# agimus-project/agimus_controller

Measured on AMD Instinct MI355X. Metric: MPC steps/sec (horizon=100, Panda 7-DoF), higher is better.
Workload: dtype f64; 1 GPU; Panda 7-DoF sine_wave_configuration_space, ocp_goal_reaching.yaml costs, horizon=100, dt=0.01, batch=1024 independent MPC instances per GPU (seed 1234+b), closed loop on own prediction; horizon=100, batch_per_gpu=1024, global_batch=1024, max_iter=10

## Files before the change

agimus_controller_amd/backend.py:

```python

from __future__ import annotations

import ctypes as C
import os
import pathlib
import subprocess

import numpy as np

from . import _abi

_CSRC = pathlib.Path(__file__).resolve().parent / "csrc"
LIB_PATH = pathlib.Path(os.environ.get("AGX_LIB", _CSRC / "libagimus_hip.so"))
NOGEN_LIB_PATH = _CSRC / "libagimus_hip_nogen.so"
_LIB = None

EXPORTED_SYMBOLS = [
    "agx_last_error", "agx_device_count", "agx_row_nref", "agx_row_nr", "agx_ref_stride",
    "agx_model_create", "agx_model_destroy", "agx_ocp_create", "agx_ocp_destroy", "agx_ocp_set_stream",
    "agx_ocp_sync", "agx_ocp_set_refs", "agx_ocp_set_refs_device", "agx_ocp_solve", "agx_ocp_upload_x0",
    "agx_ocp_upload_warmstart", "agx_ocp_solve_resident", "agx_ocp_download", "agx_ocp_download_first", "agx_ocp_first_packed", "agx_ocp_set_geom_placement", "agx_ocp_reset_duals", "agx_traj_generic_create", "agx_traj_set_horizon_indexes", "agx_ocp_feedback_rollout", "agx_ocp_download_x0", "agx_model_frame_jacobian",
    "agx_ocp_shift_warmstart", "agx_ocp_x0_from_prediction", "agx_ocp_integrate", "agx_model_rnea",
    "agx_model_frame_placement", "agx_ocp_get_residuals", "agx_ocp_calc_diff", "agx_ocp_direction",
    "agx_ocp_time_kernel", "agx_ocp_profile", "agx_traj_sine_create", "agx_traj_set_window",
    "agx_traj_get_point", "agx_traj_warmstart_from_reference", "agx_ocp_mpc_step", "agx_ocp_qp_tiles", "agx_ocp_set_quorum",
    "agx_traj_cartesian_sine_create", "agx_ocp_set_refs_async", "agx_ocp_refs_activate", "agx_ocp_refs_wait", "agx_host_alloc", "agx_host_free",
    "agx_ocp_download_async", "agx_ocp_download_wait",
    "agx_traj_generic_create_weighted", "agx_traj_cartesian_sine_wi_create", "agx_traj_get_tile",
    "agx_ocp_set_plant_inertials", "agx_model_sensitivity", "agx_ocp_cost_wide", "agx_ocp_set_model_inertials",
    "agx_traj_stream_create", "agx_traj_stream_append", "agx_traj_stream_release", "agx_traj_stream_range",
    "agx_traj_stream_joins", "agx_traj_stream_timing", "agx_ocp_set_obstacle_placements",
    "agx_ocp_set_first_pack", "agx_ocp_first_pack_counts", "agx_ocp_handoff_counts",
    "agx_ocp_iter_log", "agx_ocp_iter_log_read", "agx_ocp_item_costs", "agx_ocp_carry_counts", "agx_ocp_general_rows",
]


def _run(cmd, verbose):
    res = subprocess.run(cmd, capture_output=True, text=True)
    if verbose or res.returncode != 0:
        print(res.stdout, res.stderr)
    if res.returncode != 0:
        raise RuntimeError(f"{cmd[0]} failed ({res.returncode}): {res.stderr[-2000:]}")


def build(force: bool = False, verbose: bool = False) -> pathlib.Path:
    hdr = _CSRC.parent.parent / "include" / "agimus_hip.h"
    pairs_src = _CSRC / "agx_cost_pairs.hip"
    diag_src = _CSRC / "agx_diag.hip"
# ... 128 lines not shown
        self.nv = self.pm.nv
        self.nx, self.nu = 2 * self.nv, self.nv
        self.T, self.B = packed_ocp.horizon, int(batch)
        self.stride = packed_ocp.stride
        self.tile = _abi.tile_doubles(self.nv)
        self._log_cap = 0
        self._m = C.c_void_p()
        self._h = C.c_void_p()
        _chk(L.agx_model_create(C.byref(self.pm.desc), C.byref(self._m)))
        rc = L.agx_ocp_create(self._m, C.byref(self.po.desc), self.B, int(device), C.byref(self._h))
        if rc != 0:
            msg = L.agx_last_error().decode()
            L.agx_model_destroy(self._m)
            self._m = None
            raise HipError(msg)

    @property
    def cost_wide(self) -> bool:
        return lib().agx_ocp_cost_wide(self._h) == 1

    @property
    def general_rows(self) -> bool:
        return lib().agx_ocp_general_rows(self._h) == 1

    def close(self):
        if getattr(self, "_h", None):
            lib().agx_ocp_destroy(self._h)
            self._h = None
        if getattr(self, "_m", None):
            lib().agx_model_destroy(self._m)
# ... 95 lines not shown
        st = None
        if want_status:
            q = buf[:, nu + nk + nx:]
            names = ("kkt", "cost", "merit", "gap_norm", "iter", "qp_iters", "solved", "flags")
            if copy:
                st = np.zeros(self.B, dtype=_abi.STATUS_DTYPE)
                for k, name in enumerate(names):
                    st[name] = q[:, k] if k < 4 else q[:, k].astype(np.int32)
            else:
                st = {name: q[:, k] for k, name in enumerate(names)}
        return us0, K0, x1, st

    def set_first_pack(self, in_solve: bool = True):
        _chk(lib().agx_ocp_set_first_pack(self._h, 1 if in_solve else 0))

    def first_pack_counts(self):
        a, b = C.c_longlong(0), C.c_longlong(0)
        _chk(lib().agx_ocp_first_pack_counts(self._h, C.byref(a), C.byref(b)))
        return int(a.value), int(b.value)

    def handoff_counts(self):
        a, b = C.c_longlong(0), C.c_int(0)
        _chk(lib().agx_ocp_handoff_counts(self._h, C.byref(a), C.byref(b)))
        return int(a.value), int(b.value)

    def carry_counts(self):
        a, b = C.c_longlong(0), C.c_longlong(0)
        _chk(lib().agx_ocp_carry_counts(self._h, C.byref(a), C.byref(b)))
        return int(a.value), int(b.value)

# ... 280 lines not shown
```

agimus_controller_amd/csrc/agimus_hip.hip:

```cpp

#include <hip/hip_runtime.h>

#include <algorithm>
#include <chrono>
#include <climits>
#include <cmath>
#include <cstddef>
#include <cstdio>
#include <cstdlib>
#include <cstring>
#include <string>
#include <vector>

#include "agx_kernels.hpp"

extern "C" int agx_cost_pairs_launch(int dest, void *stream, long long nodes, const DevModel *m, const DevOcp *o, const DevCostWide *w,
                                     const double *dts, const double *xs, const RefView *rv, double *out, double *auxs, const DevState *st,
                                     int phase, int sel, int which, const void *obs);
extern "C" int agx_cost_pairs_fill_launch(void *stream, const DevCostWide *w, const double *gw_item, double *traj, long long units, int stride);
extern "C" int agx_cost_pairs_fill_ring_launch(void *stream, const DevCostWide *w, const double *gw_item, double *traj, int B, int m_new, int end,
                                               int cap, int mirror, int stride);
extern "C" int agx_diag_iter_log_launch(void *stream, const DevState *st, int B, int it, int phase, agx_iter_record *rec, int *n, int capacity);
extern "C" int agx_diag_item_costs_launch(void *stream, int nv, int chain, const DevModel *m, const DevRows *rows2, int B, int T, const double *xs,
                                          const double *us, const RefView *rv, int R, double *cost, double *Lx, double *Lu, const void *obs);
// ... 321 lines not shown
  if (kGeneralRowsWg && o->general && o->nv > 7 && !term_only) {
    const double *xs_in = phase ? o->d_xs + (size_t)o->B * (o->T + 1) * o->nx : o->d_xs;
    const double *us_in = phase ? o->d_us + (size_t)o->B * o->T * o->nu : o->d_us;
    HIPCHK((hipError_t)agx_general_rows_launch(kGenToQp, (void *)o->stream, o->nv, o->hm.prismatic ? 1 : 0, (long long)o->B * (o->T + 1), o->d_model,
                                               o->d_ocp, o->d_dt, xs_in, us_in, &o->rv, o->d_qt, o->d_aux, o->d_auxg, o->d_state, phase, -1, 0));
  }
  return o->cost_wide ? launch_cost_pairs(o, agx::kPairsToQp, running_only ? 1 : (term_only ? 2 : 0), phase) : 0;
}

template <int NV>
void launch_riccati_blk(agx_ocp *o, const double *tiles, int forward, int gains_pass) {
  hipLaunchKernelGGL((agx::k_riccati_blk<NV>), dim3(o->B), dim3(256), 0, o->stream, o->d_ocp, o->d_dt, tiles, o->d_Kws, o->d_kws, o->d_dx,
                     o->d_w, o->d_state, forward, gains_pass);
}

int launch_riccati(agx_ocp *o, int forward, bool pair = false, int iter = 0, const double *tiles = nullptr) {
  if (o->nv <= 7 && o->T + 1 > 512) return fail("the sweeps stage the step lengths of up to 511 nodes in LDS: horizon too long");
  return dispatch(o->nv, o->chain, [&](auto NVc, auto CHc) -> int {
    constexpr int NV = decltype(NVc)::value;
    const double *qt = tiles ? tiles : o->d_qt;
    if constexpr (NV <= 7) if (o->mx2_S >= 2 && o->riccati_mx && !tiles) {
      const int S = o->mx2_S, P2 = pair ? 2 : 1;
      if (!o->d_mx2_elem) {
        HIPCHK(o->own.device(&o->d_mx2_elem, 2 * (size_t)o->B * S * 768));
        HIPCHK(o->own.device(&o->d_mx2_bnd, 2 * (size_t)o->B * S * 256));
        HIPCHK(o->own.device(&o->d_mx2_cl, (size_t)o->B * S * 256));
      }
      hipLaunchKernelGGL((agx::k_riccati_mx2_elem<NV>), dim3(P2 * o->B * S), dim3(64), 0, o->stream, o->d_ocp, o->d_dt, o->d_qt, o->d_aux,
                         o->d_Kws, o->d_kws, o->d_Kout, o->d_state, o->d_mx2_elem, o->d_mx2_bnd, o->d_mx2_cl, S, pair ? 1 : 0, 0, 1, iter);
      hipLaunchKernelGGL((agx::k_riccati_mx2_sweep<NV>), dim3(P2 * o->B * (S - 1)), dim3(64), 0, o->stream, o->d_ocp, o->d_dt, o->d_qt, o->d_aux,
                         o->d_Kws, o->d_kws, o->d_Kout, o->d_state, o->d_mx2_elem, o->d_mx2_bnd, o->d_mx2_cl, S, pair ? 1 : 0, 0, 1);
      if (forward)
        hipLaunchKernelGGL((agx::k_riccati_mx2_fwd<NV>), dim3(o->B * S), dim3(64), 0, o->stream, o->d_ocp, o->d_dt, o->d_qt, o->d_Kws, o->d_kws,
                           o->d_dx, o->d_w, o->d_state, o->d_mx2_cl, S);
      HIPCHK(hipGetLastError());
      return 0;
    }
    if constexpr (NV <= 7) {
      if (pair && o->riccati_mx)
        hipLaunchKernelGGL((agx::k_riccati_mx_pair<NV>), dim3(16 * ((o->B + 7) / 8)), dim3(64), 0, o->stream, o->d_ocp, o->d_dt, o->d_qt, o->d_aux,
                           o->d_Kws, o->d_kws, o->d_dx, o->d_w, o->d_Kout, o->d_state, iter);
      else if (pair)
        hipLaunchKernelGGL((agx::k_riccati_pair<NV>), dim3(2 * o->B), dim3(64), 0, o->stream, o->d_ocp, o->d_dt, o->d_qt, o->d_aux,
                           o->d_Kws, o->d_kws, o->d_dx, o->d_w, o->d_du, o->d_Kout, o->d_state, iter);
      else if (o->riccati_mx)
        hipLaunchKernelGGL((agx::k_riccati_mx<NV, false>), dim3(o->B), dim3(64), 0, o->stream, o->d_ocp, o->d_dt, qt, o->d_aux,
                           o->d_Kws, o->d_kws, o->d_dx, o->d_w, o->d_Kout, o->d_state, forward, 0);
      else
        hipLaunchKernelGGL((agx::k_riccati<NV, false>), dim3(o->B), dim3(64), 0, o->stream, o->d_ocp, o->d_dt, qt, o->d_aux,
                           o->d_Kws, o->d_kws, o->d_dx, o->d_w, o->d_du, o->d_Kout, o->d_state, forward, 0);
    } else {
      (void)pair; (void)iter;
      launch_riccati_blk<NV>(o, qt, forward, 0);
    }
    HIPCHK(hipGetLastError());
    return 0;
  });
}

agx::HostWords host_words(agx_ocp *o, bool line_search_counters, unsigned long long seq) {
  agx::HostWords hw{nullptr, nullptr, nullptr, nullptr, nullptr, nullptr, 0};
  if (!o->poll || !o->fold_publish || seq == 0) return hw;
  hw.done = o->h_ndone_dev + 0;
  if (line_search_counters) { hw.handed = o->h_ndone_dev + 6; hw.stale = o->h_ndone_dev + 7; }
  hw.carry = o->h_ndone_dev + 8;
  hw.packed = o->h_ndone_dev + 9;
  hw.seq = o->h_ndone_dev + 1;
  hw.stamp = seq;
  return hw;
}

double *first_block(const agx_ocp *o) {
  return (o->first_in_solve && o->poll && o->first_stride == o->nu + o->nu * o->nx + o->nx + 8) ? o->d_first : nullptr;
}

int launch_step(agx_ocp *o, int iter, int max_iter, int mode, bool with_node_kkt = true, bool with_step = true, unsigned long long seq = 0,
                bool pack = false) {
  if (o->T + 1 > 512) return fail("step kernel supports horizons up to 511 nodes");
  return dispatch(o->nv, o->chain, [&](auto NVc, auto CHc) -> int {
    constexpr int NV = decltype(NVc)::value;
    constexpr bool CH = decltype(CHc)::value;
    (void)CH;
    const long long nodes = (long long)o->B * (o->T + 1);
    double *xs_t = o->d_xs + (size_t)o->B * (o->T + 1) * o->nx, *us_t = o->d_us + (size_t)o->B * o->T * o->nu;
    if (with_node_kkt) {
      if constexpr (NV <= 7) {
        if (o->general)
          hipLaunchKernelGGL((agx::k_node_kkt_gen<NV>), dim3((int)((nodes + 63) / 64)), dim3(64), 0, o->stream, o->d_ocp, o->d_qt, o->d_aux,
                             o->d_auxg, o->d_dx, o->d_w, o->d_du, o->d_nodestat, o->d_state);
        else if (o->node_kkt_wide)
          hipLaunchKernelGGL((agx::k_node_kkt_ahead<NV>), dim3((int)((nodes + 7) / 8)), dim3(64), 0, o->stream, o->d_ocp, o->d_qt, o->d_aux,
                             o->d_dx, o->d_w, o->d_du, o->d_nodestat, o->d_state);
        else
          hipLaunchKernelGGL((agx::k_node_kkt<NV>), dim3((int)((nodes * 8 + 255) / 256)), dim3(256), 0, o->stream, o->d_ocp, o->d_qt, o->d_aux,
                             o->d_dx, o->d_w, o->d_du, o->d_nodestat, o->d_state);
      } else if (kGeneralRowsWg && o->general)
        HIPCHK((hipError_t)agx_general_kkt_launch((void *)o->stream, NV, nodes, o->d_ocp, o->d_qt, o->d_aux, o->d_auxg, o->d_dx, o->d_w, o->d_du,
                                                  o->d_nodestat, o->d_state));
      else
        hipLaunchKernelGGL((agx::k_node_kkt_big<NV>), dim3((int)((nodes + 1) / 2)), dim3(64), 0, o->stream, o->d_ocp, o->d_qt, o->d_aux,
                           o->d_dx, o->d_w, o->d_du, o->d_nodestat, o->d_state);
    }
    if (with_step)
      hipLaunchKernelGGL((agx::k_sqp_head<NV>), dim3(o->B), dim3(128), 0, o->stream, o->d_ocp, o->d_xs, o->d_us, o->d_dx, o->d_du, xs_t, us_t,
                         o->d_nodestat, o->d_state, iter, max_iter, mode, o->d_ndone, host_words(o, false, seq), o->d_Kout,
                         pack ? first_block(o) : nullptr, o->first_stride);
    HIPCHK(hipGetLastError());
    return 0;
  });
}

int launch_gains(agx_ocp *o, int gmode = 0) {
  if (o->nv <= 7 && o->T + 1 > 512) return fail("the sweeps stage the step lengths of up to 511 nodes in LDS: horizon too long");
  if (o->nv > 7 && !o->d_qt2) HIPCHK(o->own.device(&o->d_qt2, (size_t)o->B * (o->T + 1) * o->qt_size));
  return dispatch(o->nv, o->chain, [&](auto NVc, auto CHc) -> int {
    constexpr int NV = decltype(NVc)::value;
    if constexpr (NV <= 7) {
      if (o->riccati_mx)
        hipLaunchKernelGGL((agx::k_riccati_mx<NV, true>), dim3(o->B), dim3(64), 0, o->stream, o->d_ocp, o->d_dt, o->d_qt, o->d_aux, o->d_Kws,
                           o->d_kws, o->d_dx, o->d_w, o->d_Kout, o->d_state, 0, gmode);
      else
// ... 398 lines not shown
    if (need_k1) {
      if (it == 0 && carry_mode != 0) {
        if (launch_calc_qp(o, false, false, 0, carry_mode == 2)) return -1;
      } else if (o->prof && it == 0) {
        if (prof_mark(o, 0, true)) return -1;
        if (launch_calc_qp(o, true, false)) return -1;
        if (prof_mark(o, 0, false)) return -1;
        if (launch_calc_qp(o, false, true)) return -1;
      } else if (launch_calc_qp(o, false, false)) return -1;
    }
    need_k1 = false;
    if (prof_mark(o, 1, true)) return -1;
    if (o->has_con && o->admm_prefactor && o->riccati_mx && o->nv <= 7 && !o->general) {
      if (admm_direction(o, true)) return -1;
    } else {
      if (launch_riccati(o, 1, pair, it)) return -1;
      if (o->has_con && admm_direction(o)) return -1;
    }
    if (prof_mark(o, 1, false)) return -1;
    const bool last = it + 1 == max_iter;
    if (prof_mark(o, 2, true)) return -1;
    const unsigned long long seq_head = ++o->seq;
    if (launch_step(o, it, max_iter, 1, !o->has_con, true, seq_head, pair && packing)) return -1;
    if (prof_mark(o, 2, false)) return -1;
    if (iter_log_mark(o, it, 0)) return -1;
    unsigned long long seq_early = 0;
    if (o->poll && !o->fold_publish && !o->prof && !o->no_empty && it >= 1) {
      seq_early = ++o->seq;
      hipLaunchKernelGGL(agx::k_publish3, dim3(1), dim3(1), 0, o->stream, o->d_ndone, o->h_ndone_dev + 11, (unsigned long long *)nullptr, (unsigned long long *)nullptr, o->h_ndone_dev + 12,
                         o->h_ndone_dev + 13, o->h_ndone_dev + 10, seq_early);
      HIPCHK(hipGetLastError());
    }
    int n_done = 0;
    if (!pair && !o->has_con && (last || max_time > 0.0 || o->quorum_sqp < 1.0)) {
      if (launch_gains(o, 4)) return -1;
    }
    bool searching = true;
    if (o->poll && o->fold_publish && it >= 1) {
// ... 780 lines not shown
    if (st) {
      const double *q = r + nu + nk + nx;
      st[b].kkt = q[0]; st[b].cost = q[1]; st[b].merit = q[2]; st[b].gap_norm = q[3];
      st[b].iter = (int)q[4]; st[b].qp_iters = (int)q[5]; st[b].solved = (int)q[6]; st[b].flags = (int)q[7];
    }
  }
  return 0;
}

int agx_ocp_set_first_pack(agx_ocp *o, int in_solve) {
  if (!o) return fail("null handle");
  o->first_in_solve = in_solve != 0;
  return 0;
}

int agx_ocp_first_pack_counts(agx_ocp *o, long long *served_in_solve, long long *served_by_launch) {
  if (!o) return fail("null handle");
  if (served_in_solve) *served_in_solve = o->first_served[0];
  if (served_by_launch) *served_by_launch = o->first_served[1];
  return 0;
}

int agx_ocp_handoff_counts(agx_ocp *o, long long *early_exits, int *n_carriable) {
  if (!o) return fail("null handle");
  if (early_exits) *early_exits = o->early_exits;
  if (n_carriable) *n_carriable = o->n_carriable;
  return 0;
}

int agx_ocp_carry_counts(agx_ocp *o, long long *steps_carried, long long *steps_full) {
// ... 302 lines not shown
  if (launch_step(o, 0, 1, 0)) return -1;
  if (launch_gains(o)) return -1;
  const size_t B = o->B, T = o->T, nx = o->nx, nu = o->nu;
  (void)nx; (void)nu;
  if (K && down_gains(o, K, o->d_Kout, B * T)) return -1;
  if (k && down(o, k, o->d_kws, B * T, 1)) return -1;
  if (dx && down(o, dx, o->d_dx, B * (T + 1), 2)) return -1;
  if (du && down(o, du, o->d_du, B * T, 1)) return -1;
  std::vector<DevState> hs(B);
  HIPCHK(hipMemcpyAsync(hs.data(), o->d_state, sizeof(DevState) * B, hipMemcpyDeviceToHost, o->stream));
  HIPCHK(hipStreamSynchronize(o->stream));
  if (kkt) for (size_t b = 0; b < B; ++b) kkt[b] = hs[b].kkt;
  return 0;
}

int agx_ocp_qp_tiles(agx_ocp *o, double *qt, double *aux, int *qt_size, int *aux_size) {
  if (!o) return fail("null handle");
  if (set_device(o)) return -1;
  if (qt_size) *qt_size = o->qt_size;
  if (aux_size) *aux_size = o->aux_size;
  if (!qt && !aux) return 0;
  if (carry_invalidate(o)) return -1;
  if (reset_state(o)) return -1;
  if (launch_calc_qp(o)) return -1;
  const size_t n = (size_t)o->B * (o->T + 1);
  if (qt) HIPCHK(hipMemcpyAsync(qt, o->d_qt, sizeof(double) * n * o->qt_size, hipMemcpyDeviceToHost, o->stream));
  if (aux) HIPCHK(hipMemcpyAsync(aux, o->d_aux, sizeof(double) * n * o->aux_size, hipMemcpyDeviceToHost, o->stream));
  HIPCHK(hipStreamSynchronize(o->stream));
  return 0;
}

#ifdef AGX_WG_PROFILE
int agx_dev_wg_stamps(long long *out, int *n) {
  int zero = 0;
  if (hipMemcpyFromSymbol(out, HIP_SYMBOL(agx::g_wg_ts), sizeof(long long) * 64) != hipSuccess) return -1;
  if (hipMemcpyFromSymbol(n, HIP_SYMBOL(agx::g_wg_n), sizeof(int)) != hipSuccess) return -1;
  (void)hipMemcpyToSymbol(HIP_SYMBOL(agx::g_wg_n), &zero, sizeof(int));
  return 0;
}
#endif

int agx_ocp_time_kernel(agx_ocp *o, int which, int reps, double *avg_ms) {
  if (!o || !avg_ms || reps < 1) return fail("agx_ocp_time_kernel: bad argument");
  if (set_device(o)) return -1;
  if (which == 10) {
    if (!o->streamed || o->st_last.buf < 0) return fail("agx_ocp_time_kernel: which = 10 needs a streamed trajectory with an append");
    HIPCHK(hipStreamSynchronize(o->stream));
    HIPCHK(hipStreamSynchronize(o->copy_stream));
    for (int pass = 0; pass < 2; ++pass) {
      if (pass == 1) HIPCHK(hipEventRecord(o->ev0, o->copy_stream));
      for (int r = 0; r < (pass == 0 ? 1 : reps); ++r)
        if (stream_enqueue_last(o, false)) return -1;
// ... 283 lines not shown
```

agimus_controller_amd/csrc/agx_host_handle.hpp:

```cpp
#pragma once

#include <deque>

namespace {

thread_local std::string g_err;
int fail(const std::string &msg) {
  g_err = msg;
  return -1;
}
#define HIPCHK(expr)                                                                                      \
  do {                                                                                                    \
    hipError_t e_ = (expr);                                                                               \
    if (e_ != hipSuccess) return fail(std::string(#expr) + ": " + hipGetErrorString(e_));                \
  } while (0)

class DeviceOwner {
 public:
  DeviceOwner() = default;
  DeviceOwner(const DeviceOwner &) = delete;
  ~DeviceOwner() { for (const Held &h : held_) free_value(*h.field, h.kind); }
  template <class T> hipError_t device(T **field, size_t count, bool zero = false) { return device_bytes((void **)field, sizeof(T) * count, zero); }
  hipError_t device_bytes(void **field, size_t bytes, bool zero = false) {
    void *p = nullptr;
// ... 75 lines not shown
         *d_fac = nullptr,
         *d_segP = nullptr;
  bool admm_segments = true;
  int qt_size = 0, aux_size = 0;
  bool k1_lanes = true;
  bool lanes_ok = true;
  bool lanes_coll = false;
  bool cost_wide = false;
  DevCostWide hw{};
  DevCostWide *d_cw = nullptr;
  DevOcp *d_ocp_k1 = nullptr;
  int n_rows_all[2] = {0, 0};
  bool speculate = true;
  bool gains_mfma = true;
  bool riccati_mx = true;
  int mx2_S = 0;
  double *d_mx2_elem = nullptr, *d_mx2_bnd = nullptr, *d_mx2_cl = nullptr;
  bool k1_fused = true;
  bool node_kkt_wide = true;
  bool tile_carry = true;
  bool carry_static = false;
  bool carry_armed = false;
  int carry_k0 = 0;
  int head = 0;
  int n_carriable = -1;
  bool frames_uniform = true;
  double quorum_sqp = 1.0, quorum_qp = 1.0;
  bool con_lanes = true;
  bool con_wide = false;
  int con_cs = AGX_MAX_NC;
// ... 179 lines not shown
```

agimus_controller_amd/csrc/agx_kernels.hpp:

```cpp
#pragma once

#include <type_traits>

#include "agx_device.hpp"

#include "agx_tiles.hpp"

namespace agx {

constexpr double kSigma = 1e-6;
constexpr double kRegMin = 1e-9;
constexpr double kRegMax = 1e9;

__device__ __forceinline__ void count_carriable(DevState &S, int *n_done) {
  const int c = (S.tiles_ok && S.preg == kRegMin) ? 1 : 0;
  if (c != S.carry_counted) { atomicAdd(n_done + 6, c - S.carry_counted); S.carry_counted = c; }
}

template <int NV, bool CHAIN, bool GEN = false, class... INST>
__global__ void __launch_bounds__(64) k_calc_diff(const DevModel *__restrict__ mp, const DevOcp *__restrict__ op,
                                                  const double *__restrict__ dts, const double *__restrict__ xs,
                                                  const double *__restrict__ us, RefView rv,
                                                  double *__restrict__ tiles, const DevState *__restrict__ st,
                                                  const INST *__restrict__... inst) {
// ... 370 lines not shown
  wave_lds_sync();
}
__device__ __forceinline__ double fast_rcp(double x) {
  double y = __builtin_amdgcn_rcp(x);
  y = y * (2.0 - x * y);
  y = y * (2.0 - x * y);
  return y;
}

template <int NV>
__device__ __forceinline__ void riccati_forward(const DevOcp &o, const int b, const int T, const double *__restrict__ dts, const double *__restrict__ qb,
                                                const double *__restrict__ Kw, const double *__restrict__ kw,
                                                double *__restrict__ dxs, double *__restrict__ wss, const double *s_dt) {
  constexpr int NX = 2 * NV, TS = QT<NV>::SIZE;
  typedef QT<NV> Q;
  const int lane = threadIdx.x;
  const int r = lane >> 3, c = lane & 7;
  const bool in = (r < NV) && (c < NV);
  const int rr = r < NV ? r : 0, cc = c < NV ? c : 0;
  const double inm = in ? 1.0 : 0.0;
  double *dx = dxs + (long long)b * (T + 1) * NX, *ws = wss + (long long)b * T * NV;
  if (lane < NV) { dx[lane] = 0.0; dx[NV + lane] = 0.0; }
  __threadfence_block();
  double dq_r = 0.0, dv_r = 0.0, dq_c = 0.0, dv_c = 0.0;
  struct Gain { double kq, kv, kw, fq, fv; };
#ifndef AGX_FWD_DEPTH
#define AGX_FWD_DEPTH 8
#endif
  constexpr int FWD_DEPTH = AGX_FWD_DEPTH;
  auto load_gain = [&](Gain &g, int t) {
    const double *kr = Kw + ((long long)t * NV + rr) * NX;
// ... 490 lines not shown
  __hip_atomic_store(hw.done, (unsigned long long)(unsigned)__hip_atomic_load(counts + 0, __ATOMIC_RELAXED, __HIP_MEMORY_SCOPE_AGENT), __ATOMIC_RELAXED, __HIP_MEMORY_SCOPE_SYSTEM);
  if (hw.handed) __hip_atomic_store(hw.handed, (unsigned long long)(unsigned)__hip_atomic_load(counts + 3, __ATOMIC_RELAXED, __HIP_MEMORY_SCOPE_AGENT), __ATOMIC_RELAXED, __HIP_MEMORY_SCOPE_SYSTEM);
  if (hw.stale) __hip_atomic_store(hw.stale, (unsigned long long)(unsigned)__hip_atomic_load(counts + 4, __ATOMIC_RELAXED, __HIP_MEMORY_SCOPE_AGENT), __ATOMIC_RELAXED, __HIP_MEMORY_SCOPE_SYSTEM);
  __hip_atomic_store(hw.carry, (unsigned long long)(unsigned)__hip_atomic_load(counts + 6, __ATOMIC_RELAXED, __HIP_MEMORY_SCOPE_AGENT), __ATOMIC_RELAXED, __HIP_MEMORY_SCOPE_SYSTEM);
  __hip_atomic_store(hw.packed, (unsigned long long)(unsigned)__hip_atomic_load(counts + 7, __ATOMIC_RELAXED, __HIP_MEMORY_SCOPE_AGENT), __ATOMIC_RELAXED, __HIP_MEMORY_SCOPE_SYSTEM);
  __threadfence_system();
  __hip_atomic_store(hw.seq, hw.stamp, __ATOMIC_RELEASE, __HIP_MEMORY_SCOPE_SYSTEM);
}

template <int NV>
__global__ void __launch_bounds__(128) k_sqp_head(const DevOcp *__restrict__ op, const double *__restrict__ xs, const double *__restrict__ us,
                                                  const double *__restrict__ dxs, const double *__restrict__ dus,
                                                  double *__restrict__ xs_t, double *__restrict__ us_t,
                                                  const double *__restrict__ nodestat, DevState *__restrict__ st, int iter, int max_iter,
                                                  int mode, int *__restrict__ n_done, HostWords hw, const double *__restrict__ Kout,
                                                  double *__restrict__ first, int first_stride) {
  __shared__ double red[8];
  __shared__ double s_words[8];
  __shared__ int flag;
  const DevOcp &o = *op;
  const int T = o.T, b = blockIdx.x, tid = threadIdx.x;
  DevState &S = st[b];
  if (S.done) {
    if (tid == 0) arrive_and_publish(n_done, hw);
    return;
  }
  constexpr int NX = 2 * NV, NU = NV;
  const int nxs = (T + 1) * NX, nus = T * NU;
  const long long ox = (long long)b * nxs, ou = (long long)b * nus;
  const bool ls = (mode & 1) && !(mode & 4);
  double px[kPrefX], pdx[kPrefX], pu[kPrefU], pdu[kPrefU];
  if (ls) {
    prefetch_strided(px, xs + ox, nxs);
    prefetch_strided(pdx, dxs + ox, nxs);
    prefetch_strided(pu, us + ou, nus);
    prefetch_strided(pdu, dus + ou, nus);
  }
  constexpr int NK = NU * NX, FS = NU + NK + NX + 8;
  const bool may_pack = first != nullptr && !o.has_con && S.gains_iter == iter;
  auto record_element = [&](int e) -> double {
    if (e < NU) return us[ou + e];
    if (e < NU + NK) return Kout[(long long)b * T * NK + (e - NU)];
    return xs[ox + NX + (e - NU - NK)];
  };
  double prec = 0.0;
  if (may_pack && tid < FS - 8) prec = record_element(tid);
  double kkt = 0.0, csum = 0.0, gsum = 0.0, vsum = 0.0;
  for (int t = tid; t <= T; t += blockDim.x) {
    const double *ns = nodestat + ((long long)b * (T + 1) + t) * 4;
    kkt = fmax(kkt, ns[0]);
    csum += ns[1];
    gsum += ns[2];
    if (o.has_con) vsum += ns[3];
  }
  kkt = wave_max(kkt);
  csum = wave_sum(csum);
  gsum = wave_sum(gsum);
  vsum = wave_sum(vsum);
  if ((tid & 63) == 0) { red[tid >> 6] = kkt; red[2 + (tid >> 6)] = csum; red[4 + (tid >> 6)] = gsum; red[6 + (tid >> 6)] = vsum; }
  __syncthreads();
  if (tid == 0) {
// ... 25 lines not shown
        S.searching = 1;
        S.ls_n = 0;
        double pr = S.preg, dr = S.dreg;
        bool stop;
        reg_schedule(1.0, pr, dr, stop);
        S.preg_trial = pr;
      }
    }
    flag = what;
    if ((mode & 1) && !(mode & 4)) count_carriable(S, n_done);
    if (what != 2) arrive_and_publish(n_done, hw);
  }
  __syncthreads();
  if (flag == 2) {
    double *rec = first + (long long)b * first_stride;
    if (tid < FS) rec[tid] = tid < FS - 8 ? prec : s_words[tid - (FS - 8)];
    for (int e = tid + blockDim.x; e < FS; e += blockDim.x)
      rec[e] = e < FS - 8 ? record_element(e) : s_words[e - (FS - 8)];
    __syncthreads();
    if (tid == 0) {
      if (hw.seq) __threadfence_system();
      atomicAdd(n_done + 7, 1);
      arrive_and_publish(n_done, hw);
    }
    return;
  }
  if (!flag) return;
#pragma unroll
  for (int k = 0; k < kPrefX; ++k) {
    const int e = tid + k * blockDim.x;
    if (e < nxs) xs_t[ox + e] = px[k] + 1.0 * pdx[k];
  }
  for (int e = tid + kPrefX * blockDim.x; e < nxs; e += blockDim.x) xs_t[ox + e] = xs[ox + e] + 1.0 * dxs[ox + e];
// ... 921 lines not shown
```

agimus_controller_amd/csrc/agx_riccati_mx.hpp:

```cpp
#pragma once

namespace agx {

typedef double mx4 __attribute__((ext_vector_type(4)));
typedef __attribute__((address_space(3))) double lds_double;

#ifndef AGX_MX_DEPTH
#define AGX_MX_DEPTH 4
#endif
constexpr int kMxDepth = AGX_MX_DEPTH;

template <int K>
__device__ __forceinline__ double row_bcast(double x) { return __builtin_amdgcn_mov_dpp(x, 0x150 + K, 0xf, 0xf, false); }
__device__ __forceinline__ double row_ror8(double x) {
  const int lo = __double2loint(x), hi = __double2hiint(x);
  return __hiloint2double(__builtin_amdgcn_mov_dpp(hi, 0x128, 0xf, 0xf, false), __builtin_amdgcn_mov_dpp(lo, 0x128, 0xf, 0xf, false));
}
__device__ __forceinline__ double chain_rcp(double x) {
  const double y0 = __builtin_amdgcn_rcp(x);
  const double e = __builtin_fma(-x, y0, 1.0);
  const double y1 = __builtin_fma(y0, e, y0), e2 = e * e;
  return __builtin_fma(y1, e2, y1);
}
__device__ __forceinline__ double flip_sign(double x) { return __hiloint2double(__double2hiint(x) ^ (int)0x80000000, __double2loint(x)); }

template <int NV, bool GAINS, bool CLOOP, bool ELEM, class TLo>
__device__ __forceinline__ void riccati_mx_seg(const int b, const DevOcp *__restrict__ op, const double *__restrict__ dts,
                                               const double *__restrict__ qts, const double *__restrict__ auxs,
                                               double *__restrict__ Kws, double *__restrict__ kws, double *__restrict__ Kout,
                                               const double dreg, const TLo t_lo_, const int t_hi, const int vinit, mx4 &Vio, mx4 &Am,
                                               mx4 &At, mx4 &Cm, bool &bad, lds_double *s_dt) {
  static_assert(NV <= 7, "16-column tiles: 7 joints + the gradient slot per half");
  typedef QT<NV> Q;
  typedef AUX<NV> A;
  constexpr int NX = 2 * NV, TS = Q::SIZE, LD = Q::LD;
  constexpr int Z = Q::cost + 1;
  const DevOcp &o = *op;
  const int T = o.T, lane = threadIdx.x, t_lo = t_lo_;
  const double sig = GAINS ? kSigma : 0.0;
  const double *qb = qts + (long long)b * (T + 1) * TS;
  const double *ab = auxs + (long long)b * (T + 1) * A::SIZE;

  const int j = lane & 15, g = lane >> 4;
  auto xreal = [](int X) { return (X & 7) < NV; };
  auto xoff = [](int X) { return X < 8 ? X : NV + (X - 8); };
  int oHxx[4], oHwx[2], oHww[2], oF[4], oTx[2], oMt[2];
  double mTx[2], mMt[2];
#pragma unroll
  for (int r = 0; r < 4; ++r) {
    const int i = g + 4 * r;
    int off = Z;
    if (xreal(i)) {
      if (j == 7) off = GAINS ? Z : Q::gx + xoff(i);
// ... 73 lines not shown
    }
  };

  mx4 V;
  if (vinit == 1) {
    const double *tt = qb + (long long)T * TS;
#pragma unroll
    for (int r = 0; r < 4; ++r) V[r] = tt[oHxx[r]] + dg[r];
  } else if (vinit == 0) {
#pragma unroll
    for (int r = 0; r < 4; ++r) V[r] = 0.0;
  } else {
    V = Vio;
  }
  bool bad_pivot = false;
  if constexpr (CLOOP) {
#pragma unroll
    for (int r = 0; r < 4; ++r) { Am[r] = 2.0 * ih[r]; At[r] = 2.0 * ih[r]; Cm[r] = 0.0; }
  }

  auto step = [&](Tile &z, int t) {
    const double h = s_dt[t], h2 = h * h;
    double Hxx[4] = {z.hxx[0], z.hxx[1], z.hxx[2], z.hxx[3]};
    double Hwx[2] = {z.hwx[0], z.hwx[1]}, Hww[2] = {z.hww[0], z.hww[1]};
    double Tx[2] = {0.0, 0.0}, Mt[2] = {0.0, 0.0};
    if (GAINS) {
      Tx[0] = z.tx[0] * mTx[0]; Tx[1] = z.tx[1] * mTx[1]; Mt[0] = z.mt[0] * mMt[0]; Mt[1] = z.mt[1] * mMt[1];
      const double sT0 = sig * Tx[0], sT1 = sig * Tx[1], sM0 = sig * Mt[0], sM1 = sig * Mt[1];
      mx4 hx = {Hxx[0], Hxx[1], Hxx[2], Hxx[3]};
      hx = __builtin_amdgcn_mfma_f64_16x16x4f64(sT0, Tx[0], hx, 0, 0, 0);
// ... 85 lines not shown
        Cm = __builtin_amdgcn_mfma_f64_16x16x4f64(GAt[0], Z0, Cm, 0, 0, 0);
        Cm = __builtin_amdgcn_mfma_f64_16x16x4f64(GAt[1], Z1, Cm, 0, 0, 0);
      }
      Am = An; At = Atn;
    }
    if constexpr (ELEM) {
    } else if (!GAINS) {
      if (stV[0]) stP[0][(long long)t * stK[0]] = K0;
      if (stV[1]) stP[1][(long long)t * stK[1]] = K1;
    } else {
      mx4 ku = {flip_sign(Tx[0]), flip_sign(Tx[1]), 0.0, 0.0};
      ku = __builtin_amdgcn_mfma_f64_16x16x4f64(Mt[0], K0, ku, 0, 0, 0);
      ku = __builtin_amdgcn_mfma_f64_16x16x4f64(Mt[1], K1, ku, 0, 0, 0);
      if (stV[0]) stP[0][(long long)t * stK[0]] = ku[0];
      if (stV[1]) stP[1][(long long)t * stK[1]] = ku[1];
    }
    prefetch_group_begin();
    load_tile(z, t - kMxDepth >= t_lo ? t - kMxDepth : t_lo);
    prefetch_group_end();
  };

  int t = t_hi - 1;
  for (int r = (t_hi - t_lo) % kMxDepth; r > 0; --r, --t) {
    Tile z;
    load_tile(z, t);
    step(z, t);
  }
  if (t >= t_lo) {
    Tile tl[kMxDepth];
#pragma unroll
    for (int i = 0; i < kMxDepth; ++i) load_tile(tl[i], t - i);
    prefetch_queue_settle(tl);
    for (; t >= t_lo; t -= kMxDepth) {
#pragma unroll
      for (int i = 0; i < kMxDepth; ++i) step(tl[i], t - i);
    }
  }
  Vio = V;
  bad = bad_pivot;
}

template <int NV, bool GAINS>
__device__ __forceinline__ void riccati_mx_body(const int b, const DevOcp *op, const double *dts, const double *qts, const double *auxs,
                                                double *Kws, double *kws, double *__restrict__ dxs, double *__restrict__ wss,
                                                double *Kout, DevState *__restrict__ st, int forward, int gmode, int iter) {
  constexpr int NX = 2 * NV, TS = QT<NV>::SIZE;
  const DevOcp &o = *op;
  const int T = o.T, lane = threadIdx.x;
  DevState &S = st[b];
  if (!GAINS && (S.done || S.admm_conv)) return;
  if (GAINS && (gmode == 1 || gmode == 4) && S.done) return;
  if (GAINS && gmode == 2 && S.gains_iter == S.dir_iter) return;
  const double dreg = (GAINS && gmode != 1 && gmode != 4) ? (S.solved ? S.dreg : S.gains_dreg) : S.dreg;
  if (GAINS && gmode != 0 && lane == 0) S.gains_iter = (gmode == 1) ? iter : S.dir_iter;
  __shared__ double s_dt[kMaxHorizon];
  mx4 V, Am, At, Cm;
  bool bad_pivot = false;
  riccati_mx_seg<NV, GAINS, false, false>(b, op, dts, qts, auxs, Kws, kws, Kout, dreg, std::integral_constant<int, 0>(), T,  1, V, Am, At, Cm, bad_pivot, (lds_double *)s_dt);
  if (!GAINS) {
    const bool any_bad = __any(bad_pivot);
    if (lane == 0) {
      if (gmode != 3) S.dir_fail = any_bad ? 1 : 0;
      if (any_bad) atomicOr(&S.flags, 1);
    }
  }
  if (GAINS || !forward) return;
  const double *qb = qts + (long long)b * (T + 1) * TS;
  riccati_forward<NV>(o, b, T, dts, qb, Kws + (long long)b * T * NV * NX, kws + (long long)b * T * NV, dxs, wss, s_dt);
}

template <int NV, bool GAINS>
__global__ void __launch_bounds__(64, 2) k_riccati_mx(const DevOcp *__restrict__ op, const double *__restrict__ dts,
                                                   const double *__restrict__ qts, const double *__restrict__ auxs,
                                                   double *__restrict__ Kws, double *__restrict__ kws, double *__restrict__ dxs,
                                                   double *__restrict__ wss, double *__restrict__ Kout, DevState *__restrict__ st,
                                                   int forward, int gmode) {
  riccati_mx_body<NV, GAINS>(blockIdx.x, op, dts, qts, auxs, Kws, kws, dxs, wss, Kout, st, forward, gmode, 0);
}

template <int NV>
__global__ void __launch_bounds__(64, 2) k_riccati_mx_pair(const DevOcp *__restrict__ op, const double *__restrict__ dts,
                                                        const double *__restrict__ qts, const double *__restrict__ auxs,
                                                        double *__restrict__ Kws, double *__restrict__ kws, double *__restrict__ dxs,
                                                        double *__restrict__ wss, double *__restrict__ Kout, DevState *__restrict__ st,
                                                        int iter) {
  const int grp = blockIdx.x >> 4, w16 = blockIdx.x & 15;
  const int b = grp * 8 + (w16 & 7);
  if (b >= op->B) return;
  if (w16 >> 3)
    riccati_mx_body<NV, true>(b, op, dts, qts, auxs, Kws, kws, dxs, wss, Kout, st, 0, 1, iter);
  else
    riccati_mx_body<NV, false>(b, op, dts, qts, auxs, Kws, kws, dxs, wss, Kout, st, 1, 0, iter);
}

}
```

include/agimus_hip.h:

```cpp
#ifndef AGIMUS_HIP_H
#define AGIMUS_HIP_H

#include <stddef.h>
#include <stdint.h>

#ifdef __cplusplus
extern "C" {
#endif

#define AGX_MAX_ROWS 8
#define AGX_MAX_COST_PAIRS 64
#define AGX_MAX_NV 32
#define AGX_JOINT_REVOLUTE 0
#define AGX_JOINT_PRISMATIC 1

enum agx_residual_kind {
  AGX_RES_STATE = 0,
  AGX_RES_CONTROL = 1,
  AGX_RES_CONTROL_GRAV = 2,
  AGX_RES_FRAME_PLACEMENT = 3,
  AGX_RES_FRAME_TRANSLATION = 4,
  AGX_RES_FRAME_ROTATION = 5,
  AGX_RES_FRAME_VELOCITY = 6,
  AGX_RES_COLLISION = 7
// ... 116 lines not shown
int agx_ocp_set_refs_device(agx_ocp *ocp, const double *d_ref_tile, const int32_t *d_frame_ids, int adopt);

int agx_ocp_solve(agx_ocp *ocp, const double *x0, const double *xs_ws, const double *us_ws,
                  int max_iter, double max_time, double *xs, double *us, double *K, agx_status *st);

int agx_ocp_upload_x0(agx_ocp *ocp, const double *x0);
int agx_ocp_upload_warmstart(agx_ocp *ocp, const double *xs_ws, const double *us_ws);
int agx_ocp_solve_resident(agx_ocp *ocp, int max_iter, double max_time);
int agx_ocp_download(agx_ocp *ocp, double *xs, double *us, double *K, agx_status *st);
int agx_ocp_download_async(agx_ocp *ocp, double *xs, double *us, double *K);
int agx_ocp_download_wait(agx_ocp *ocp);
int agx_ocp_download_first(agx_ocp *ocp, double *us0, double *K0, double *x1, agx_status *st);
int agx_ocp_first_packed(agx_ocp *ocp, const double **host, int *stride);
int agx_ocp_set_first_pack(agx_ocp *ocp, int in_solve);
int agx_ocp_first_pack_counts(agx_ocp *ocp, long long *served_in_solve, long long *served_by_launch);
int agx_ocp_handoff_counts(agx_ocp *ocp, long long *early_exits, int *n_carriable);
int agx_ocp_carry_counts(agx_ocp *ocp, long long *steps_carried, long long *steps_full);

int agx_ocp_shift_warmstart(agx_ocp *ocp);
int agx_ocp_x0_from_prediction(agx_ocp *ocp);

int agx_ocp_integrate(agx_ocp *ocp, int n, const double *x, const double *u, double *xnext);

int agx_model_rnea(agx_ocp *ocp, int n, const double *q, const double *v, const double *a, double *tau);
int agx_model_frame_placement(agx_ocp *ocp, int n, int frame, const double *q, double *out);
int agx_model_frame_jacobian(agx_ocp *ocp, int n, int frame, int local, const double *q, double *J);

int agx_model_sensitivity(agx_ocp *ocp, int n, double dt, const double *x, const double *u,
                          double delta_inertia, double delta_com, double delta_mass, double *out);

// ... 58 lines not shown
```

Baseline: 1.299 million MPC steps/s.

## Write first-node gains from the paired Riccati sweep; add optional 8-wave workgroup variant

The gains half of the paired Riccati kernel now records the first-node feedback gain K0 straight into the packed first-step record. The step-head kernel then skips re-reading and re-writing those K0 entries, which cuts global traffic on the packing path. An opt-in 512-thread kernel is also added that puts four instances' direction and gains sweeps in one workgroup with per-wave LDS step-length buffers, plus debug and census hooks. The workgroup variant is off by default. The K0 path adds a cross-kernel dependency on when the first record is written.

```diff
diff --git a/agimus_controller_amd/backend.py b/agimus_controller_amd/backend.py
--- a/agimus_controller_amd/backend.py
+++ b/agimus_controller_amd/backend.py
@@ -32,6 +32,7 @@
     "agx_traj_stream_joins", "agx_traj_stream_timing", "agx_ocp_set_obstacle_placements",
     "agx_ocp_set_first_pack", "agx_ocp_first_pack_counts", "agx_ocp_handoff_counts",
     "agx_ocp_iter_log", "agx_ocp_iter_log_read", "agx_ocp_item_costs", "agx_ocp_carry_counts", "agx_ocp_general_rows",
+    "agx_ocp_set_pair_wg", "agx_ocp_debug_sweeps",
 ]
 
 
@@ -190,6 +191,8 @@
             L.agx_model_destroy(self._m)
             self._m = None
             raise HipError(msg)
+        if "AGX_PAIR_WG" in os.environ:
+            self.set_pair_wg(os.environ["AGX_PAIR_WG"][:1] != "0")
 
     @property
     def cost_wide(self) -> bool:
@@ -315,6 +318,18 @@
     def set_first_pack(self, in_solve: bool = True):
         _chk(lib().agx_ocp_set_first_pack(self._h, 1 if in_solve else 0))
 
+    def set_pair_wg(self, eight_waves: bool):
+        _chk(lib().agx_ocp_set_pair_wg(self._h, 1 if eight_waves else 0))
+
+    def debug_sweeps(self, paired: bool, done=()):
+        cap = C.c_int(0)
+        _chk(lib().agx_ocp_debug_sweeps(self._h, 0, None, 0, C.byref(cap), None, None, None, None, None))
+        n, B, T = cap.value, self.B, self.T
+        out = [np.empty((B, T + 1, 2 * n)), np.empty((B, T, n)), np.empty((B, T, n, 2 * n)), np.empty((B, T, n)), np.empty((B, T, n, 2 * n))]
+        d = np.ascontiguousarray(np.asarray(list(done), dtype=np.int32))
+        _chk(lib().agx_ocp_debug_sweeps(self._h, 1 if paired else 0, d.ctypes.data_as(C.c_void_p), int(d.size), C.byref(cap), *[_p(a) for a in out]))
+        return tuple(out)
+
     def first_pack_counts(self):
         a, b = C.c_longlong(0), C.c_longlong(0)
         _chk(lib().agx_ocp_first_pack_counts(self._h, C.byref(a), C.byref(b)))
diff --git a/agimus_controller_amd/csrc/agimus_hip.hip b/agimus_controller_amd/csrc/agimus_hip.hip
--- a/agimus_controller_amd/csrc/agimus_hip.hip
+++ b/agimus_controller_amd/csrc/agimus_hip.hip
@@ -359,7 +359,15 @@
                      o->d_w, o->d_state, forward, gains_pass);
 }
 
-int launch_riccati(agx_ocp *o, int forward, bool pair = false, int iter = 0, const double *tiles = nullptr) {
+double *first_block(const agx_ocp *o) {
+  return (o->first_in_solve && o->poll && o->first_stride == o->nu + o->nu * o->nx + o->nx + 8) ? o->d_first : nullptr;
+}
+
+bool k0_by_sweep(const agx_ocp *o, bool pair) {
+  return pair && first_block(o) != nullptr && o->nv <= 7 && o->riccati_mx && o->mx2_S < 2;
+}
+
+int launch_riccati(agx_ocp *o, int forward, bool pair = false, int iter = 0, const double *tiles = nullptr, double *first = nullptr) {
   if (o->nv <= 7 && o->T + 1 > 512) return fail("the sweeps stage the step lengths of up to 511 nodes in LDS: horizon too long");
   return dispatch(o->nv, o->chain, [&](auto NVc, auto CHc) -> int {
     constexpr int NV = decltype(NVc)::value;
@@ -382,9 +390,12 @@
       return 0;
     }
     if constexpr (NV <= 7) {
-      if (pair && o->riccati_mx)
+      if (pair && o->riccati_mx && o->pair_wg)
+        hipLaunchKernelGGL((agx::k_riccati_mx_pair_wg<NV>), dim3((o->B + 3) / 4), dim3(512), 0, o->stream, o->d_ocp, o->d_dt, o->d_qt, o->d_aux,
+                           o->d_Kws, o->d_kws, o->d_dx, o->d_w, o->d_Kout, o->d_state, iter, first, o->first_stride);
+      else if (pair && o->riccati_mx)
         hipLaunchKernelGGL((agx::k_riccati_mx_pair<NV>), dim3(16 * ((o->B + 7) / 8)), dim3(64), 0, o->stream, o->d_ocp, o->d_dt, o->d_qt, o->d_aux,
-                           o->d_Kws, o->d_kws, o->d_dx, o->d_w, o->d_Kout, o->d_state, iter);
+                           o->d_Kws, o->d_kws, o->d_dx, o->d_w, o->d_Kout, o->d_state, iter, first, o->first_stride);
       else if (pair)
         hipLaunchKernelGGL((agx::k_riccati_pair<NV>), dim3(2 * o->B), dim3(64), 0, o->stream, o->d_ocp, o->d_dt, o->d_qt, o->d_aux,
                            o->d_Kws, o->d_kws, o->d_dx, o->d_w, o->d_du, o->d_Kout, o->d_state, iter);
@@ -415,12 +426,8 @@
   return hw;
 }
 
-double *first_block(const agx_ocp *o) {
-  return (o->first_in_solve && o->poll && o->first_stride == o->nu + o->nu * o->nx + o->nx + 8) ? o->d_first : nullptr;
-}
-
 int launch_step(agx_ocp *o, int iter, int max_iter, int mode, bool with_node_kkt = true, bool with_step = true, unsigned long long seq = 0,
-                bool pack = false) {
+                bool pack = false, bool k0_there = false) {
   if (o->T + 1 > 512) return fail("step kernel supports horizons up to 511 nodes");
   return dispatch(o->nv, o->chain, [&](auto NVc, auto CHc) -> int {
     constexpr int NV = decltype(NVc)::value;
@@ -449,7 +456,7 @@
     if (with_step)
       hipLaunchKernelGGL((agx::k_sqp_head<NV>), dim3(o->B), dim3(128), 0, o->stream, o->d_ocp, o->d_xs, o->d_us, o->d_dx, o->d_du, xs_t, us_t,
                          o->d_nodestat, o->d_state, iter, max_iter, mode, o->d_ndone, host_words(o, false, seq), o->d_Kout,
-                         pack ? first_block(o) : nullptr, o->first_stride);
+                         pack ? first_block(o) : nullptr, o->first_stride, pack && k0_there ? 1 : 0);
     HIPCHK(hipGetLastError());
     return 0;
   });
@@ -878,14 +885,14 @@
     if (o->has_con && o->admm_prefactor && o->riccati_mx && o->nv <= 7 && !o->general) {
       if (admm_direction(o, true)) return -1;
     } else {
-      if (launch_riccati(o, 1, pair, it)) return -1;
+      if (launch_riccati(o, 1, pair, it, nullptr, k0_by_sweep(o, pair) ? first_block(o) : nullptr)) return -1;
       if (o->has_con && admm_direction(o)) return -1;
     }
     if (prof_mark(o, 1, false)) return -1;
     const bool last = it + 1 == max_iter;
     if (prof_mark(o, 2, true)) return -1;
     const unsigned long long seq_head = ++o->seq;
-    if (launch_step(o, it, max_iter, 1, !o->has_con, true, seq_head, pair && packing)) return -1;
+    if (launch_step(o, it, max_iter, 1, !o->has_con, true, seq_head, pair && packing, k0_by_sweep(o, pair))) return -1;
     if (prof_mark(o, 2, false)) return -1;
     if (iter_log_mark(o, it, 0)) return -1;
     unsigned long long seq_early = 0;
@@ -1696,6 +1703,12 @@
   return 0;
 }
 
+int agx_ocp_set_pair_wg(agx_ocp *o, int eight_waves) {
+  if (!o) return fail("null handle");
+  o->pair_wg = eight_waves != 0;
+  return 0;
+}
+
 int agx_ocp_first_pack_counts(agx_ocp *o, long long *served_in_solve, long long *served_by_launch) {
   if (!o) return fail("null handle");
   if (served_in_solve) *served_in_solve = o->first_served[0];
@@ -2028,6 +2041,43 @@
   return 0;
 }
 
+int agx_ocp_debug_sweeps(agx_ocp *o, int paired, const int *done, int n_done, int *nv_cap, double *dx, double *w, double *Kws, double *kws,
+                         double *Kout) {
+  if (!o) return fail("null handle");
+  if (nv_cap) *nv_cap = o->nv;
+  if (!dx && !w && !Kws && !kws && !Kout) return 0;
+  if (o->nv > 7 || !o->riccati_mx || o->has_con) return fail("agx_ocp_debug_sweeps: unconstrained models of up to 7 joints on the MFMA-layout sweeps");
+  if (set_device(o)) return -1;
+  if (carry_invalidate(o)) return -1;
+  if (reset_state(o)) return -1;
+  if (launch_calc_qp(o)) return -1;
+  const size_t B = o->B, T = o->T, nx = o->nx, nu = o->nu;
+  if (n_done > 0) {
+    std::vector<DevState> hs(B);
+    HIPCHK(hipMemcpyAsync(hs.data(), o->d_state, sizeof(DevState) * B, hipMemcpyDeviceToHost, o->stream));
+    HIPCHK(hipStreamSynchronize(o->stream));
+    for (int i = 0; i < n_done; ++i) {
+      if (done[i] < 0 || done[i] >= o->B) return fail("agx_ocp_debug_sweeps: instance out of range");
+      hs[done[i]].done = 1;
+    }
+    HIPCHK(hipMemcpyAsync(o->d_state, hs.data(), sizeof(DevState) * B, hipMemcpyHostToDevice, o->stream));
+    HIPCHK(hipStreamSynchronize(o->stream));
+  }
+  struct { double *host, *dev; size_t n; } arr[5] = {{dx, o->d_dx, B * (T + 1) * nx}, {w, o->d_w, B * T * nu}, {Kws, o->d_Kws, B * T * nu * nx},
+                                                     {kws, o->d_kws, B * T * nu}, {Kout, o->d_Kout, B * T * nu * nx}};
+  for (auto &a : arr) HIPCHK(hipMemsetAsync(a.dev, 0, sizeof(double) * a.n, o->stream));
+  if (paired) {
+    if (launch_riccati(o, 1, true, 1)) return -1;
+  } else {
+    if (launch_riccati(o, 1, false)) return -1;
+    if (launch_gains(o, 1)) return -1;
+  }
+  for (auto &a : arr)
+    if (a.host) HIPCHK(hipMemcpyAsync(a.host, a.dev, sizeof(double) * a.n, hipMemcpyDeviceToHost, o->stream));
+  HIPCHK(hipStreamSynchronize(o->stream));
+  return 0;
+}
+
 int agx_ocp_qp_tiles(agx_ocp *o, double *qt, double *aux, int *qt_size, int *aux_size) {
   if (!o) return fail("null handle");
   if (set_device(o)) return -1;
@@ -2050,6 +2100,18 @@
   if (hipMemcpyFromSymbol(out, HIP_SYMBOL(agx::g_wg_ts), sizeof(long long) * 64) != hipSuccess) return -1;
   if (hipMemcpyFromSymbol(n, HIP_SYMBOL(agx::g_wg_n), sizeof(int)) != hipSuccess) return -1;
   (void)hipMemcpyToSymbol(HIP_SYMBOL(agx::g_wg_n), &zero, sizeof(int));
+  return 0;
+}
+#endif
+
+#ifdef AGX_PAIR_CENSUS
+extern "C" int agx_dev_pair_census(unsigned long long *out, int *n_slots) {
+  const size_t bytes = sizeof(unsigned long long) * 8 * agx::kCensusSlots;
+  if (hipDeviceSynchronize() != hipSuccess) return -1;
+  if (hipMemcpyFromSymbol(out, HIP_SYMBOL(agx::g_pair_census), bytes) != hipSuccess) return -1;
+  std::vector<unsigned long long> zero(8 * agx::kCensusSlots, 0ull);
+  if (hipMemcpyToSymbol(HIP_SYMBOL(agx::g_pair_census), zero.data(), bytes) != hipSuccess) return -1;
+  *n_slots = agx::kCensusSlots;
   return 0;
 }
 #endif
diff --git a/agimus_controller_amd/csrc/agx_host_handle.hpp b/agimus_controller_amd/csrc/agx_host_handle.hpp
--- a/agimus_controller_amd/csrc/agx_host_handle.hpp
+++ b/agimus_controller_amd/csrc/agx_host_handle.hpp
@@ -113,6 +113,7 @@
   bool speculate = true;
   bool gains_mfma = true;
   bool riccati_mx = true;
+  bool pair_wg = false;
   int mx2_S = 0;
   double *d_mx2_elem = nullptr, *d_mx2_bnd = nullptr, *d_mx2_cl = nullptr;
   bool k1_fused = true;
diff --git a/agimus_controller_amd/csrc/agx_kernels.hpp b/agimus_controller_amd/csrc/agx_kernels.hpp
--- a/agimus_controller_amd/csrc/agx_kernels.hpp
+++ b/agimus_controller_amd/csrc/agx_kernels.hpp
@@ -408,7 +408,7 @@
                                                 double *__restrict__ dxs, double *__restrict__ wss, const double *s_dt) {
   constexpr int NX = 2 * NV, TS = QT<NV>::SIZE;
   typedef QT<NV> Q;
-  const int lane = threadIdx.x;
+  const int lane = threadIdx.x & 63;
   const int r = lane >> 3, c = lane & 7;
   const bool in = (r < NV) && (c < NV);
   const int rr = r < NV ? r : 0, cc = c < NV ? c : 0;
@@ -929,7 +929,7 @@
                                                   double *__restrict__ xs_t, double *__restrict__ us_t,
                                                   const double *__restrict__ nodestat, DevState *__restrict__ st, int iter, int max_iter,
                                                   int mode, int *__restrict__ n_done, HostWords hw, const double *__restrict__ Kout,
-                                                  double *__restrict__ first, int first_stride) {
+                                                  double *__restrict__ first, int first_stride, int k0_there) {
   __shared__ double red[8];
   __shared__ double s_words[8];
   __shared__ int flag;
@@ -958,8 +958,9 @@
     if (e < NU + NK) return Kout[(long long)b * T * NK + (e - NU)];
     return xs[ox + NX + (e - NU - NK)];
   };
+  auto packed_here = [&](int e) { return !(k0_there && e >= NU && e < NU + NK); };
   double prec = 0.0;
-  if (may_pack && tid < FS - 8) prec = record_element(tid);
+  if (may_pack && tid < FS - 8 && packed_here(tid)) prec = record_element(tid);
   double kkt = 0.0, csum = 0.0, gsum = 0.0, vsum = 0.0;
   for (int t = tid; t <= T; t += blockDim.x) {
     const double *ns = nodestat + ((long long)b * (T + 1) + t) * 4;
@@ -1015,9 +1016,9 @@
   __syncthreads();
   if (flag == 2) {
     double *rec = first + (long long)b * first_stride;
-    if (tid < FS) rec[tid] = tid < FS - 8 ? prec : s_words[tid - (FS - 8)];
+    if (tid < FS && packed_here(tid)) rec[tid] = tid < FS - 8 ? prec : s_words[tid - (FS - 8)];
     for (int e = tid + blockDim.x; e < FS; e += blockDim.x)
-      rec[e] = e < FS - 8 ? record_element(e) : s_words[e - (FS - 8)];
+      if (packed_here(e)) rec[e] = e < FS - 8 ? record_element(e) : s_words[e - (FS - 8)];
     __syncthreads();
     if (tid == 0) {
       if (hw.seq) __threadfence_system();
diff --git a/agimus_controller_amd/csrc/agx_riccati_mx.hpp b/agimus_controller_amd/csrc/agx_riccati_mx.hpp
--- a/agimus_controller_amd/csrc/agx_riccati_mx.hpp
+++ b/agimus_controller_amd/csrc/agx_riccati_mx.hpp
@@ -29,14 +29,14 @@
                                                const double *__restrict__ qts, const double *__restrict__ auxs,
                                                double *__restrict__ Kws, double *__restrict__ kws, double *__restrict__ Kout,
                                                const double dreg, const TLo t_lo_, const int t_hi, const int vinit, mx4 &Vio, mx4 &Am,
-                                               mx4 &At, mx4 &Cm, bool &bad, lds_double *s_dt) {
+                                               mx4 &At, mx4 &Cm, bool &bad, lds_double *s_dt, double *k0rec = nullptr) {
   static_assert(NV <= 7, "16-column tiles: 7 joints + the gradient slot per half");
   typedef QT<NV> Q;
   typedef AUX<NV> A;
   constexpr int NX = 2 * NV, TS = Q::SIZE, LD = Q::LD;
   constexpr int Z = Q::cost + 1;
   const DevOcp &o = *op;
-  const int T = o.T, lane = threadIdx.x, t_lo = t_lo_;
+  const int T = o.T, lane = threadIdx.x & 63, t_lo = t_lo_;
   const double sig = GAINS ? kSigma : 0.0;
   const double *qb = qts + (long long)b * (T + 1) * TS;
   const double *ab = auxs + (long long)b * (T + 1) * A::SIZE;
@@ -140,6 +140,7 @@
     V = Vio;
   }
   bool bad_pivot = false;
+  double ku_last[2] = {0.0, 0.0};
   if constexpr (CLOOP) {
 #pragma unroll
     for (int r = 0; r < 4; ++r) { Am[r] = 2.0 * ih[r]; At[r] = 2.0 * ih[r]; Cm[r] = 0.0; }
@@ -255,6 +256,7 @@
       ku = __builtin_amdgcn_mfma_f64_16x16x4f64(Mt[1], K1, ku, 0, 0, 0);
       if (stV[0]) stP[0][(long long)t * stK[0]] = ku[0];
       if (stV[1]) stP[1][(long long)t * stK[1]] = ku[1];
+      ku_last[0] = ku[0]; ku_last[1] = ku[1];
     }
     prefetch_group_begin();
     load_tile(z, t - kMxDepth >= t_lo ? t - kMxDepth : t_lo);
@@ -277,27 +279,37 @@
       for (int i = 0; i < kMxDepth; ++i) step(tl[i], t - i);
     }
   }
+  if constexpr (GAINS && !ELEM) {
+    if (k0rec != nullptr && t_lo == 0) {
+#pragma unroll
+      for (int s = 0; s < 2; ++s) {
+        const int w = g + 4 * s;
+        if ((w < NV) && xreal(j) && j != 7) k0rec[w * NX + xoff(j)] = ku_last[s];
+      }
+    }
+  }
   Vio = V;
   bad = bad_pivot;
 }
+
 
 template <int NV, bool GAINS>
 __device__ __forceinline__ void riccati_mx_body(const int b, const DevOcp *op, const double *dts, const double *qts, const double *auxs,
                                                 double *Kws, double *kws, double *__restrict__ dxs, double *__restrict__ wss,
-                                                double *Kout, DevState *__restrict__ st, int forward, int gmode, int iter) {
+                                                double *Kout, DevState *__restrict__ st, int forward, int gmode, int iter, double *s_dt,
+                                                double *k0rec = nullptr) {
   constexpr int NX = 2 * NV, TS = QT<NV>::SIZE;
   const DevOcp &o = *op;
-  const int T = o.T, lane = threadIdx.x;
+  const int T = o.T, lane = threadIdx.x & 63;
   DevState &S = st[b];
   if (!GAINS && (S.done || S.admm_conv)) return;
   if (GAINS && (gmode == 1 || gmode == 4) && S.done) return;
   if (GAINS && gmode == 2 && S.gains_iter == S.dir_iter) return;
   const double dreg = (GAINS && gmode != 1 && gmode != 4) ? (S.solved ? S.dreg : S.gains_dreg) : S.dreg;
   if (GAINS && gmode != 0 && lane == 0) S.gains_iter = (gmode == 1) ? iter : S.dir_iter;
-  __shared__ double s_dt[kMaxHorizon];
   mx4 V, Am, At, Cm;
   bool bad_pivot = false;
-  riccati_mx_seg<NV, GAINS, false, false>(b, op, dts, qts, auxs, Kws, kws, Kout, dreg, std::integral_constant<int, 0>(), T,  1, V, Am, At, Cm, bad_pivot, (lds_double *)s_dt);
+  riccati_mx_seg<NV, GAINS, false, false>(b, op, dts, qts, auxs, Kws, kws, Kout, dreg, std::integral_constant<int, 0>(), T,  1, V, Am, At, Cm, bad_pivot, (lds_double *)s_dt, k0rec);
   if (!GAINS) {
     const bool any_bad = __any(bad_pivot);
     if (lane == 0) {
@@ -308,6 +320,14 @@
   if (GAINS || !forward) return;
   const double *qb = qts + (long long)b * (T + 1) * TS;
   riccati_forward<NV>(o, b, T, dts, qb, Kws + (long long)b * T * NV * NX, kws + (long long)b * T * NV, dxs, wss, s_dt);
+}
+
+template <int NV, bool GAINS>
+__device__ __forceinline__ void riccati_mx_body(const int b, const DevOcp *op, const double *dts, const double *qts, const double *auxs,
+                                                double *Kws, double *kws, double *__restrict__ dxs, double *__restrict__ wss,
+                                                double *Kout, DevState *__restrict__ st, int forward, int gmode, int iter) {
+  __shared__ double s_dt[kMaxHorizon];
+  riccati_mx_body<NV, GAINS>(b, op, dts, qts, auxs, Kws, kws, dxs, wss, Kout, st, forward, gmode, iter, s_dt);
 }
 
 template <int NV, bool GAINS>
@@ -316,22 +336,74 @@
                                                    double *__restrict__ Kws, double *__restrict__ kws, double *__restrict__ dxs,
                                                    double *__restrict__ wss, double *__restrict__ Kout, DevState *__restrict__ st,
                                                    int forward, int gmode) {
-  riccati_mx_body<NV, GAINS>(blockIdx.x, op, dts, qts, auxs, Kws, kws, dxs, wss, Kout, st, forward, gmode, 0);
-}
+  __shared__ double s_dt[kMaxHorizon];
+  riccati_mx_body<NV, GAINS>(blockIdx.x, op, dts, qts, auxs, Kws, kws, dxs, wss, Kout, st, forward, gmode, 0, s_dt);
+}
+
+#ifdef AGX_PAIR_CENSUS
+constexpr int kCensusSlots = 4096;
+__device__ unsigned long long g_pair_census[8 * kCensusSlots];
+struct PairCensus {
+  unsigned long long t0, r0;
+  __device__ __forceinline__ PairCensus() : t0(__builtin_amdgcn_s_memtime()), r0(__builtin_amdgcn_s_memrealtime()) {}
+  __device__ __forceinline__ void leave(int slot, int role, int b) const {
+    const unsigned long long t1 = __builtin_amdgcn_s_memtime(), r1 = __builtin_amdgcn_s_memrealtime();
+    if ((threadIdx.x & 63) == 0 && slot < kCensusSlots) {
+      unsigned long long *e = g_pair_census + 8 * slot;
+      e[0] = __builtin_amdgcn_s_getreg(4 | (31 << 11));
+      e[1] = __builtin_amdgcn_s_getreg(20 | (31 << 11));
+      e[2] = (unsigned long long)role | ((unsigned long long)b << 8);
+      e[3] = t0; e[4] = t1; e[5] = r0; e[6] = r1; e[7] = 1;
+    }
+  }
+};
+#endif
 
 template <int NV>
 __global__ void __launch_bounds__(64, 2) k_riccati_mx_pair(const DevOcp *__restrict__ op, const double *__restrict__ dts,
                                                         const double *__restrict__ qts, const double *__restrict__ auxs,
                                                         double *__restrict__ Kws, double *__restrict__ kws, double *__restrict__ dxs,
                                                         double *__restrict__ wss, double *__restrict__ Kout, DevState *__restrict__ st,
-                                                        int iter) {
+                                                        int iter, double *first, int first_stride) {
+  __shared__ double s_dt[kMaxHorizon];
   const int grp = blockIdx.x >> 4, w16 = blockIdx.x & 15;
   const int b = grp * 8 + (w16 & 7);
   if (b >= op->B) return;
+#ifdef AGX_PAIR_CENSUS
+  const PairCensus census;
+#endif
   if (w16 >> 3)
-    riccati_mx_body<NV, true>(b, op, dts, qts, auxs, Kws, kws, dxs, wss, Kout, st, 0, 1, iter);
+    riccati_mx_body<NV, true>(b, op, dts, qts, auxs, Kws, kws, dxs, wss, Kout, st, 0, 1, iter, s_dt,
+                              first ? first + (long long)b * first_stride + NV : nullptr);
   else
-    riccati_mx_body<NV, false>(b, op, dts, qts, auxs, Kws, kws, dxs, wss, Kout, st, 1, 0, iter);
-}
-
-}
+    riccati_mx_body<NV, false>(b, op, dts, qts, auxs, Kws, kws, dxs, wss, Kout, st, 1, 0, iter, s_dt);
+#ifdef AGX_PAIR_CENSUS
+  census.leave(blockIdx.x, w16 >> 3, b);
+#endif
+}
+
+template <int NV>
+__global__ void __launch_bounds__(512) k_riccati_mx_pair_wg(const DevOcp *__restrict__ op, const double *__restrict__ dts,
+                                                            const double *__restrict__ qts, const double *__restrict__ auxs,
+                                                            double *__restrict__ Kws, double *__restrict__ kws,
+                                                            double *__restrict__ dxs, double *__restrict__ wss,
+                                                            double *__restrict__ Kout, DevState *__restrict__ st, int iter,
+                                                            double *first, int first_stride) {
+  __shared__ double s_dt[8 * kMaxHorizon];
+  const int wave = __builtin_amdgcn_readfirstlane(threadIdx.x >> 6);
+  const int b = blockIdx.x * 4 + (wave & 3);
+  if (b >= op->B) return;
+#ifdef AGX_PAIR_CENSUS
+  const PairCensus census;
+#endif
+  if (wave >> 2)
+    riccati_mx_body<NV, true>(b, op, dts, qts, auxs, Kws, kws, dxs, wss, Kout, st, 0, 1, iter, s_dt + wave * kMaxHorizon,
+                              first ? first + (long long)b * first_stride + NV : nullptr);
+  else
+    riccati_mx_body<NV, false>(b, op, dts, qts, auxs, Kws, kws, dxs, wss, Kout, st, 1, 0, iter, s_dt + wave * kMaxHorizon);
+#ifdef AGX_PAIR_CENSUS
+  census.leave(8 * blockIdx.x + wave, wave >> 2, b);
+#endif
+}
+
+}
diff --git a/include/agimus_hip.h b/include/agimus_hip.h
--- a/include/agimus_hip.h
+++ b/include/agimus_hip.h
@@ -154,6 +154,9 @@
 int agx_ocp_first_packed(agx_ocp *ocp, const double **host, int *stride);
 int agx_ocp_set_first_pack(agx_ocp *ocp, int in_solve);
 int agx_ocp_first_pack_counts(agx_ocp *ocp, long long *served_in_solve, long long *served_by_launch);
+int agx_ocp_set_pair_wg(agx_ocp *ocp, int eight_waves);
+int agx_ocp_debug_sweeps(agx_ocp *ocp, int paired, const int *done, int n_done, int *nv_cap, double *dx, double *w, double *Kws,
+                         double *kws, double *Kout);
 int agx_ocp_handoff_counts(agx_ocp *ocp, long long *early_exits, int *n_carriable);
 int agx_ocp_carry_counts(agx_ocp *ocp, long long *steps_carried, long long *steps_full);
 
```

Result: no change. 1.315 million MPC steps/s (median of 3 runs) (+1.3%).
